# dnbaker/bonsai

Hardware: AMD Instinct MI355X
Metric: reads/s classified (150 bp) (higher is better)
Workload: dtype u64

## Files before the change

### bonsai_amd/csrc/bns_device.hpp

```cpp
#pragma once
#include <hip/hip_runtime.h>
#include <stdint.h>
#include <type_traits>

namespace bns {

using u8 = uint8_t;
using u16 = uint16_t;
using u32 = uint32_t;
using u64 = uint64_t;

constexpr u32 TAX_ABSENT = 0xFFFFFFFFu;

struct alignas(16) Slot {
    u64 key;
    u32 val;
    u32 occ;
};

struct alignas(16) TaxNode {
    u32 parent;
    u32 tin, tout;
    u32 flags;
};
constexpr u32 NODE_PRESENT = 1u, NODE_CHAIN_OK = 2u;

__device__ __forceinline__ int lane_id() { return (int)(threadIdx.x & 63u); }

__device__ __forceinline__ u64 wang64(u64 key)
{
    key = (~key) + (key << 21);
    key = key ^ (key >> 24);
    key = (key + (key << 3)) + (key << 8);
    key = key ^ (key >> 14);
    key = (key + (key << 2)) + (key << 4);
    key = key ^ (key >> 28);
    key = key + (key << 31);
    return key;
}

__device__ __forceinline__ u32 pairswap_not(u32 x)
{
    u32 r;
    const u32 c = 0x55555555u;
    asm("v_bitop3_b32 %0, %1, %2, %3 bitop3:0x1b" : "=v"(r) : "v"(x >> 1), "v"(x << 1), "s"(c));
    return r;
}
__device__ __forceinline__ u64 revcomp(u64 kmer, u32 k)
{
    const u32 a = __builtin_bitreverse32((u32)(kmer >> 32)), b = __builtin_bitreverse32((u32)kmer);
    const u32 lo = pairswap_not(a), hi = pairswap_not(b);
    return (((u64)hi << 32) | lo) >> (64u - (k << 1));
}

__device__ __forceinline__ u64 revcomp_top(u64 win, u32 k)
{
    const u32 a = __builtin_bitreverse32((u32)(win >> 32)), b = __builtin_bitreverse32((u32)win);
    const u32 lo = pairswap_not(a), hi = pairswap_not(b);
    return (((u64)hi << 32) | lo) & (~0ULL >> (64u - (k << 1)));
}

__device__ __forceinline__ u64 canonical(u64 kmer, u32 k)
{
    const u64 rc = revcomp(kmer, k);
    return kmer < rc ? kmer : rc;
}

template <int CTRL>
__device__ __forceinline__ u32 dpp(u32 v)
{
    return (u32)__builtin_amdgcn_update_dpp(0, (int)v, CTRL, 0xf, 0xf, true);
}
template <int CTRL>
__device__ __forceinline__ u64 dpp64(u64 v)
{
    const u32 lo = dpp<CTRL>((u32)v), hi = dpp<CTRL>((u32)(v >> 32));
    return ((u64)hi << 32) | lo;
}
constexpr int QP_XOR1 = 0xB1;
constexpr int QP_XOR2 = 0x4E;
template <int S> struct QBcast { static constexpr int ctrl = S * 0x55; };

__device__ __forceinline__ u64 ballot64(bool p) { return __builtin_amdgcn_ballot_w64(p); }
__device__ __forceinline__ u32 readlane(u32 v, int l) { return (u32)__builtin_amdgcn_readlane((int)v, l); }
__device__ __forceinline__ u64 readlane64(u64 v, int l)
{
    return ((u64)readlane((u32)(v >> 32), l) << 32) | readlane((u32)v, l);
}
__device__ __forceinline__ u64 lanemask_lt() { return (1ULL << lane_id()) - 1ULL; }

struct ProbeResult { u32 val; bool found; };
#ifdef BNS_COUNT_FETCHES
__device__ unsigned long long g_fetch_count[8];
#endif

__device__ __forceinline__ ProbeResult probe_khash(const u32 *__restrict__ flags, const u64 *__restrict__ keys,
                                                   const u32 *__restrict__ vals, u64 n_buckets, u64 key, bool active)
{
    ProbeResult r{0u, false};
    if (!active || n_buckets == 0) return r;
    const u64 mask = n_buckets - 1;
    u64 i = wang64(key) & mask, step = 0;
    const u64 last = i;
    for (;;) {
        const u32 f = (flags[i >> 4] >> ((i & 0xfu) << 1)) & 3u;
        if (f & 2u) return r;
        if (!(f & 1u) && keys[i] == key) { r.val = vals[i]; r.found = true; return r; }
        i = (i + (++step)) & mask;
        if (i == last) return r;
    }
}

// ... 293 lines not shown
    if (!PEEL || pass(std::true_type{}))
        while (more && pass(std::false_type{})) {}
#ifdef BNS_COUNT_FETCHES
    { const u64 g2 = ballot64(found == 2u); if (g2 && lane == 0) { atomicAdd(&g_fetch_count[2], (unsigned long long)__popcll(g2)); atomicAdd(&g_fetch_count[3], 1ULL); } }
#endif
    if (OVF_COOP) {
        bool go = found == 2u;
        u64 todo = ballot64(go);
        if (todo) {
            u32 *lb = aux, *lstep = aux + 16, *lres = aux + 32, *lflag = aux + 48;
            u64 *lkey = reinterpret_cast<u64 *>(aux + MINB_LIST_U32);
            const uint4 *ob = reinterpret_cast<const uint4 *>(ovf_slots);
            u32 l3 = (u32)lane;
            asm volatile("" : "+v"(l3));
            const u32 q = (l3 >> 2) & 15u, sub = l3 & 3u;
            do {
                const u32 rank = __builtin_amdgcn_mbcnt_hi((u32)(todo >> 32), __builtin_amdgcn_mbcnt_lo((u32)todo, 0u));
                const bool mine = go && rank < 16u;
                const u32 n = (u32)__popcll(todo);
                if (mine) { lkey[rank] = key; lb[rank] = (u32)ovf_bucket(key, ovf_mask); lstep[rank] = 0u; lflag[rank] = 0u; }
                __builtin_amdgcn_wave_barrier();
                bool walking = q < n;
                while (ballot64(walking)) {
                    u32 b = 0;
                    uint4 sl = make_uint4(0u, 0u, 0u, 0u);
                    if (walking) { b = lb[q]; sl = ob[(u64)b * 4u + sub]; }
                    const bool occ = sl.w != 0u;
                    const bool match = walking && occ && ((((u64)sl.y << 32) | sl.x) == lkey[q]);
                    u32 mv = match ? sl.z : 0u, fl = (match ? 1u : 0u) | (occ ? 2u : 0u);
                    mv |= dpp<QP_XOR1>(mv); mv |= dpp<QP_XOR2>(mv);
                    { const u32 o1 = dpp<QP_XOR1>(fl); fl = ((fl | o1) & 1u) | (fl & o1 & 2u); }
                    { const u32 o2 = dpp<QP_XOR2>(fl); fl = ((fl | o2) & 1u) | (fl & o2 & 2u); }
                    if (walking && sub == 0u) {
                        if (fl & 1u) { lres[q] = mv; lflag[q] = 1u; }
                        else if (fl & 2u) { const u32 st = lstep[q] + 1u; lstep[q] = st; lb[q] = (u32)(((u64)b + st) & ovf_mask); }
                    }
                    walking = walking && fl == 2u;
                    __builtin_amdgcn_wave_barrier();
                }
                if (mine && lflag[rank]) { found = 1u; val = lres[rank]; }
                go = go && !mine;
                todo = ballot64(go);
                __builtin_amdgcn_wave_barrier();
            } while (todo);
        }
        return ProbeResult{val, (found & 1u) != 0u};
    }
    minb_ovf_walk(key, found, val, ovf_slots, ovf_mask);
    ProbeResult r{val, (found & 1u) != 0u};
    return r;
}

constexpr int MINB_NB_WIDE = 24;
template <bool KEY_MAY_BE_ONES = true, int NB = 16>
__device__ __forceinline__ void probe_minbucket2(const MinBucket *__restrict__ buckets, u64 keyA, u32 bA, bool activeA, u64 keyB, u32 bB,
                                                 bool activeB, u32 *aux, const Slot *__restrict__ ovf_slots, u64 ovf_mask,
                                                 ProbeResult &ra, ProbeResult &rb, u32 nb = 16u)
{
    static_assert(NB == 16, "the two-key probe is built on a 16-bucket stage (two 1 KiB loads; nb = 24 adds a third)");
    const int lane = lane_id();
    u32 *list = aux;
    uint4 *stage = reinterpret_cast<uint4 *>(aux + MINB_LIST_U32);
    const uint4 *base = reinterpret_cast<const uint4 *>(buckets);
    u32 bktA = activeA ? bA : MINB_NONE, bktB = activeB ? bB : MINB_NONE;
    u32 foundA = 0u, valA = 0u, homeA = 0u, foundB = 0u, valB = 0u, homeB = 0u;
    const u32 xfA = mph_fold(keyA), xfB = mph_fold(keyB);
    constexpr u32 GO = 1u << MINB_HOME_SHIFT;
    auto look = [&](auto first_tag, u32 &bkt, u32 rank, u32 xf, u64 key, u32 &found, u32 &val, u32 home, u32 &hx) -> bool {
        constexpr bool FIRST = decltype(first_tag)::value;
        const bool mine = bkt != MINB_NONE && rank < nb;
        const char *B = reinterpret_cast<const char *>(stage) + (mine ? rank : 0u) * (16u * MINB_STRIDE);
        const uint2 hdr = *reinterpret_cast<const uint2 *>(B + 120);
        const u32 slot = mph_slot(xf, hdr.y);
        const bool eq = *reinterpret_cast<const u64 *>(B + 8u * slot) == key;
        const bool hit = mine & eq & (!KEY_MAY_BE_ONES || ((hdr.x >> (8u + slot)) & 1u));
        const u32 v = *reinterpret_cast<const u32 *>(B + 80 + 4u * slot);
        found = hit ? 1u : found;
        val = hit ? v : val;
        bool cont;
        if (FIRST) cont = mine & !hit & ((hdr.x & (GO | 0xFFu)) >= (GO | MINB_CAP));
        else       cont = mine & !hit & ((hdr.x & 0xFFu) >= MINB_CAP) & ((((home ? home : hdr.x) & GO)) != 0u);
        bkt = (mine && !cont) ? MINB_NONE : bkt;
        hx = hdr.x;
        return cont;
    };
    auto walk = [&](auto first_tag, bool cont, u32 hx, u32 &bkt, u32 &found, u32 &home) {
        constexpr bool FIRST = decltype(first_tag)::value;
        const u32 cur = (FIRST || home == 0u) ? ((hx & MINB_HOME_MASK) | (GO << 4)) : home;
        const bool exhausted = cont && (cur >> (MINB_HOME_SHIFT + 2u)) == 0u;
        found |= (exhausted || (cont && (hx & 0xFFu) == MINB_N_IN_OVF)) ? 2u : 0u;
        const u32 next = exhausted ? MINB_NONE : bkt + 1u;
        bkt = cont ? next : bkt;
        home = cont ? cur >> 1 : home;
    };
    bool more = true;
#ifdef BNS_COUNT_FETCHES
    u32 why_later = 4u;
#endif
    auto pass = [&](auto first_tag) -> bool {
        const u32 a63 = readlane(bktA, 63);
        const u32 prevA = (u32)__builtin_amdgcn_update_dpp((int)~bktA, (int)bktA, DPP_WAVE_SHR1, 0xf, 0xf, false);
        const u32 prevB = (u32)__builtin_amdgcn_update_dpp((int)a63, (int)bktB, DPP_WAVE_SHR1, 0xf, 0xf, false);
        const bool pendA = bktA != MINB_NONE, chgA = bktA != prevA, pendB = bktB != MINB_NONE, chgB = bktB != prevB;
        const u64 leadA = ballot64(pendA) & ballot64(chgA), leadB = ballot64(pendB) & ballot64(chgB);
        if (!(leadA | leadB)) return false;
        const u32 nA = (u32)__popcll(leadA);
        const int n_lead = (int)nA + __popcll(leadB);
#ifdef BNS_COUNT_FETCHES
        if (lane == 0) {
            atomicAdd(&g_fetch_count[0], (unsigned long long)((u32)n_lead < nb ? (u32)n_lead : nb)); atomicAdd(&g_fetch_count[1], 1ULL);
            if (!decltype(first_tag)::value) atomicAdd(&g_fetch_count[why_later], 1ULL);
        }
#endif
        const u32 rankA = __builtin_amdgcn_mbcnt_hi((u32)(leadA >> 33), __builtin_amdgcn_mbcnt_lo((u32)(leadA >> 1), (u32)(leadA & 1ULL) - 1u));
        const u32 rankB = __builtin_amdgcn_mbcnt_hi((u32)(leadB >> 33), __builtin_amdgcn_mbcnt_lo((u32)(leadB >> 1), nA + (u32)(leadB & 1ULL) - 1u));
        if (pendA & chgA) list[rankA] = bktA;
        if ((pendB & chgB) && rankB < nb) list[rankB] = bktB;
        __builtin_amdgcn_wave_barrier();
        {
            const u32 last = (u32)n_lead - 1u, slot = (u32)lane >> 3;
            typedef const void __attribute__((address_space(1))) *gptr_t;
            typedef void __attribute__((address_space(3))) *lptr_t;
            const u32 b0 = list[slot < last ? slot : last];
            __builtin_amdgcn_global_load_lds((gptr_t)(base + ((u64)b0 * 8 + (u64)(lane & 7))), (lptr_t)stage, 16, 0, 2);
            if (last >= 8u) {
                const u32 b1 = list[slot + 8u < last ? slot + 8u : last];
                __builtin_amdgcn_global_load_lds((gptr_t)(base + ((u64)b1 * 8 + (u64)(lane & 7))), (lptr_t)(stage + 64), 16, 0, 2);
                if (last >= 16u && nb > 16u) {
                    const u32 b2 = list[slot + 16u < last ? slot + 16u : last];
                    __builtin_amdgcn_global_load_lds((gptr_t)(base + ((u64)b2 * 8 + (u64)(lane & 7))), (lptr_t)(stage + 128), 16, 0, 2);
                }
            }
            asm volatile("s_waitcnt vmcnt(0)" ::: "memory");
        }
        __builtin_amdgcn_wave_barrier();
        u32 hxA, hxB;
        const bool contA = look(first_tag, bktA, rankA, xfA, keyA, foundA, valA, homeA, hxA);
        const bool contB = look(first_tag, bktB, rankB, xfB, keyB, foundB, valB, homeB, hxB);
        const u64 cA = ballot64(contA), cB = ballot64(contB);
        more = (u32)n_lead > nb || (cA | cB) != 0ULL;
#ifdef BNS_COUNT_FETCHES
        why_later = 4u + ((u32)n_lead > nb ? 1u : 0u) + ((cA | cB) != 0ULL ? 2u : 0u);
#endif
        if (cA) walk(first_tag, contA, hxA, bktA, foundA, homeA);
        if (cB) walk(first_tag, contB, hxB, bktB, foundB, homeB);
        __builtin_amdgcn_wave_barrier();
        return true;
    };
    if (pass(std::true_type{}))
        while (more && pass(std::false_type{})) {}
#ifdef BNS_COUNT_FETCHES
    { const u64 gA = ballot64(foundA == 2u), gB = ballot64(foundB == 2u);
      if ((gA | gB) && lane == 0) { atomicAdd(&g_fetch_count[2], (unsigned long long)(__popcll(gA) + __popcll(gB))); atomicAdd(&g_fetch_count[3], 1ULL); } }
#endif
    minb_ovf_walk(keyA, foundA, valA, ovf_slots, ovf_mask);
    minb_ovf_walk(keyB, foundB, valB, ovf_slots, ovf_mask);
    ra = ProbeResult{valA, (foundA & 1u) != 0u};
    rb = ProbeResult{valB, (foundB & 1u) != 0u};
}

__device__ __forceinline__ TaxNode load_node(const TaxNode *__restrict__ nodes, u32 n_nodes, u32 id)
{
    if (id < n_nodes) return nodes[id];
    return TaxNode{TAX_ABSENT, 0u, 0u, 0u};
}

__device__ __forceinline__ bool anc_or_self(u32 x, const TaxNode &nx, u32 a, const TaxNode &na)
{
    return x == a || (nx.tin < na.tin && na.tin < nx.tout);
// ... 20 lines not shown
```

### bonsai_amd/csrc/bns_kernels.hip

```cpp
#include "bns_device.hpp"
#include "bns_kernels.hpp"

namespace bns {

typedef const volatile __attribute__((address_space(4))) ClassifyParams ColdParams;
__device__ __forceinline__ ColdParams *cold_params() { return (ColdParams *)__builtin_amdgcn_kernarg_segment_ptr(); }

__device__ __forceinline__ u32 base_code(u32 b, u32 &bad)
{
    const u32 c = b & 0xDFu;
    const bool ok = (c == 0x41u) | (c == 0x43u) | (c == 0x47u) | (c == 0x54u);
    const u32 x = (c >> 1) & 3u;
    bad = ok ? 0u : 1u;
    return ok ? (x ^ (x >> 1)) : 0u;
}

__global__ __launch_bounds__(256) void pack_kernel(const u8 *__restrict__ bases, const u64 *__restrict__ offsets,
                                                   u64 n_reads, u64 *__restrict__ words, u32 *__restrict__ nmask)
{
    const int lane = lane_id();
    const u64 wave = (u64)blockIdx.x * (blockDim.x >> 6) + (u64)__builtin_amdgcn_readfirstlane((int)(threadIdx.x >> 6));
    const u64 n_waves = (u64)gridDim.x * (blockDim.x >> 6);
    for (u64 r = wave; r < n_reads; r += n_waves) {
        const u64 o = offsets[r];
// ... 111 lines not shown
    if (PACKED) asm volatile("" : "+v"(f.lo), "+v"(f.hi), "+v"(f.m));
    else        asm volatile("" : "+v"(f.lo), "+v"(f.hi));
}
template <bool PACKED>
__device__ __forceinline__ void prefetch_issue(const ClassifyParams &p, u64 r, u64 o, u32 L, Prefetch &f)
{
    if (!PACKED) { raw_load<true>(p.bases, o, L, 0u, f.lo, f.hi); return; }
    const u32 lane = (u32)lane_id();
    if (lane < ((L + 31u) >> 5)) {
        const u64 wi = (o >> 5) + r + lane;
        const u64 w = p.words[wi];
        f.lo = (u32)w; f.hi = (u32)(w >> 32);
        if (p.nmask) f.m = p.nmask[wi];
    }
}
__device__ __forceinline__ u64 mask1_to_mask2(u32 m)
{
    u64 x = m;
    x = (x | (x << 16)) & 0x0000FFFF0000FFFFULL;
    x = (x | (x << 8)) & 0x00FF00FF00FF00FFULL;
    x = (x | (x << 4)) & 0x0F0F0F0F0F0F0F0FULL;
    x = (x | (x << 2)) & 0x3333333333333333ULL;
    x = (x | (x << 1)) & 0x5555555555555555ULL;
    return x * 3ULL;
}
template <bool ORD32 = false>
__device__ __forceinline__ bool load_chunk_packed(const ClassifyParams &p, u64 r, u64 o, u32 L, u32 j0, bool have, const Prefetch &f, u64 *pk)
{
    const u32 lane = (u32)lane_id();
    u64 w = ((u64)f.hi << 32) | f.lo;
    u32 m = f.m;
    if (!have) {
        w = 0; m = 0;
        const u32 wl = (j0 >> 5) + lane;
        if (wl < ((L + 31u) >> 5)) {
            const u64 wi = (o >> 5) + r + wl;
            w = p.words[wi];
            if (p.nmask) m = p.nmask[wi];
        }
    }
    const bool dirty = ballot64(m != 0u) != 0ULL;
    if (ORD32) {
        u32 *img = reinterpret_cast<u32 *>(pk);
        img[1u + 2u * lane] = (u32)(w >> 32); img[2u + 2u * lane] = (u32)w;
        if (dirty) { const u64 m2 = mask1_to_mask2(m); img[IMG_N32 + 1u + 2u * lane] = (u32)(m2 >> 32); img[IMG_N32 + 2u + 2u * lane] = (u32)m2; }
    } else {
        pk[lane] = w;
        if (dirty) pk[64 + lane] = mask1_to_mask2(m);
    }
    __builtin_amdgcn_wave_barrier();
    return !dirty;
}

__device__ __forceinline__ void extract_lds32(const u64 *pk, u32 rd, u32 k, bool clean, u64 &win, bool &valid)
{
    const u32 lane = (u32)lane_id();
    const u32 *img = reinterpret_cast<const u32 *>(pk);
    const u32 g = 4u * rd + ((lane + 15u) >> 4), n = 30u - 2u * ((lane + 15u) & 15u);
    const u32 w0 = img[g], w1 = img[g + 1u], w2 = img[g + 2u];
    const u32 hi = __builtin_amdgcn_alignbit(w0, w1, n), lo = __builtin_amdgcn_alignbit(w1, w2, n);
    win = ((u64)hi << 32) | lo;
    valid = true;
    if (!clean) {
        const u32 m0 = img[IMG_N32 + g], m1 = img[IMG_N32 + g + 1u], m2 = img[IMG_N32 + g + 2u];
        const u64 mw = ((u64)__builtin_amdgcn_alignbit(m0, m1, n) << 32) | __builtin_amdgcn_alignbit(m1, m2, n);
        valid = (mw >> (64u - 2u * k)) == 0;
    }
}

__device__ __forceinline__ u32 mask2_to_mask1(u64 m2)
{
    u64 x = m2 & 0x5555555555555555ULL;
    x = (x | (x >> 1)) & 0x3333333333333333ULL;
    x = (x | (x >> 2)) & 0x0F0F0F0F0F0F0F0FULL;
    x = (x | (x >> 4)) & 0x00FF00FF00FF00FFULL;
    x = (x | (x >> 8)) & 0x0000FFFF0000FFFFULL;
    x = (x | (x >> 16)) & 0x00000000FFFFFFFFULL;
    return (u32)x;
}

__device__ __forceinline__ bool extract_unspaced(u64 W, u32 M, u32 rd, u32 k, u64 &kmer)
{
    const int lane = lane_id();
    const int w0 = (int)(2 * rd);
    const u64 wa = readlane64(W, w0), wb = readlane64(W, w0 + 1), wc = readlane64(W, w0 + 2);
    const u32 ma = readlane(M, w0), mb = readlane(M, w0 + 1), mc = readlane(M, w0 + 2);
    const bool up = lane >= 32;
    const u64 hi = up ? wb : wa, lo = up ? wc : wb;
    const u64 m64 = up ? (((u64)mb << 32) | mc) : (((u64)ma << 32) | mb);
    const u32 o = (u32)lane & 31u;
    const u64 win = o ? ((hi << (2 * o)) | (lo >> (64 - 2 * o))) : hi;
    kmer = win >> (64u - 2u * k);
    return ((m64 << o) >> (64u - k)) == 0;
}

template <int CTRL>
__device__ __forceinline__ u32 dpp_keep(u32 v)
{
    return (u32)__builtin_amdgcn_update_dpp(-1, (int)v, CTRL, 0xf, 0xf, false);
}
__device__ __forceinline__ u32 row_prefix_min(u32 x)
{
    x = min(x, dpp_keep<0x111>(x)); x = min(x, dpp_keep<0x112>(x)); x = min(x, dpp_keep<0x114>(x)); x = min(x, dpp_keep<0x118>(x));
    return x;
}
__device__ __forceinline__ u32 row_suffix_min(u32 x)
{
    x = min(x, dpp_keep<0x101>(x)); x = min(x, dpp_keep<0x102>(x)); x = min(x, dpp_keep<0x104>(x)); x = min(x, dpp_keep<0x108>(x));
    return x;
}
__device__ __forceinline__ u32 window16_min(u32 mine, u32 head, u32 rd, u32 *ring)
{
    const u32 lane = (u32)lane_id();
    if (rd == 0) {
        asm volatile("");
        const u32 sh = row_suffix_min(lane < 15u ? head : 0xFFFFFFFFu);
        if (lane < 15u) ring[lane] = sh;
    }
    const u32 P = row_prefix_min(mine), S = row_suffix_min(mine);
    ring[15u + lane] = S;
    __builtin_amdgcn_wave_barrier();
    const u32 sprev = ring[lane];
    __builtin_amdgcn_wave_barrier();
    if (lane >= 49u) ring[lane - 49u] = S;
    return min(P, sprev);
}

template <int W, bool VH = false>
__device__ __forceinline__ u32 round_minhash(u64 kf, u64 rc, u32 rd, u32 k, u32 m, u32 *ring)
{
    const int lane = lane_id();
    const u32 span = k - m;
    const u64 mmask = ~0ULL >> (64u - 2u * m);
    if (span == 0) { const u64 a = kf & mmask, b = rc & mmask; return mmer_hash(a < b ? a : b); }
    u32 mine;
    if (VH) {
        u32 head = 0;
        if (m <= 16u) {
            const u32 mm = 0xFFFFFFFFu >> (32u - 2u * m);
            if (rd == 0) head = mmer_mix(min((u32)(kf >> 30) & mm, (u32)rc & mm));
            mine = mmer_mix(min((u32)kf & mm, (u32)(rc >> 30)));
        } else {
            if (rd == 0) { const u64 a = kf >> 30, b = rc & mmask; head = mmer_hash(a < b ? a : b); }
            const u64 a = kf & mmask, b = rc >> 30;
            mine = mmer_hash(a < b ? a : b);
        }
        return window16_min(mine, head, rd, ring);
    }
    if (m <= 16u) {
        const u32 mm = 0xFFFFFFFFu >> (32u - 2u * m);
        if (rd == 0) { asm volatile(""); if ((u32)lane < span) ring[lane] = mmer_mix(min((u32)(kf >> (2u * span)) & mm, (u32)rc & mm)); }
        mine = mmer_mix(min((u32)kf & mm, (u32)(rc >> (2u * span))));
        ring[span + (u32)lane] = mine;
    } else {
        if (rd == 0) {
            if ((u32)lane < span) {
                const u64 a = kf >> (2u * span), b = rc & mmask;
                ring[lane] = mmer_hash(a < b ? a : b);
            }
        }
        const u64 a = kf & mmask, b = rc >> (2u * span);
        mine = mmer_hash(a < b ? a : b);
        ring[span + (u32)lane] = mine;
    }
    __builtin_amdgcn_wave_barrier();
    constexpr u32 G = W <= 9 ? (u32)W : ((u32)W + 1u) / 2u;
    u32 best = 0xFFFFFFFFu;
#pragma unroll
    for (u32 g = 0; g < (u32)W; g += G) {
        u32 h[G + 1];
#pragma unroll
        for (u32 i = 0; i <= G; ++i) h[i] = (i < G && g + i < (u32)W) ? ring[(u32)lane + g + i] : 0xFFFFFFFFu;
        if (span == (u32)W - 1u) {
#pragma unroll
            for (u32 i = 0; i < G; i += 2) if (g + i < (u32)W) best = min(min(best, h[i]), h[i + 1]);
        } else {
#pragma unroll
            for (u32 i = 0; i < G; ++i) { const u32 x = g + i <= span ? h[i] : 0xFFFFFFFFu; best = x < best ? x : best; }
        }
        if (g + G < (u32)W) { asm volatile("" : "+v"(best)); __builtin_amdgcn_sched_barrier(0); }
    }
    __builtin_amdgcn_wave_barrier();
    if ((u32)lane >= 64u - span) ring[(u32)lane + span - 64u] = mine;
    return best;
}

template <int W>
__device__ __forceinline__ u64 round_minhash_wide(u64 kf, u64 rc, u32 rd, u32 k, u32 m, u64 *ring)
{
    const int lane = lane_id();
    const u32 span = k - m;
    const u64 mmask = ~0ULL >> (64u - 2u * m);
    u64 mine;
    if (m <= 16u) {
        const u32 mm = 0xFFFFFFFFu >> (32u - 2u * m);
        if (span && rd == 0 && (u32)lane < span) ring[lane] = wide_ident32(min((u32)(kf >> (2u * span)) & mm, (u32)rc & mm));
        mine = wide_ident32(min((u32)kf & mm, (u32)(rc >> (2u * span)) & mm));
    } else {
        if (span && rd == 0 && (u32)lane < span) { const u64 a = kf >> (2u * span), b = rc & mmask; ring[lane] = wide_ident64(a < b ? a : b); }
        const u64 a = kf & mmask, b = rc >> (2u * span);
// ... 331 lines not shown
        best = s > best ? s : best;
    }
#pragma unroll
    for (int off = 32; off >= 1; off >>= 1) {
        const u32 o = (u32)__shfl_xor((int)best, off);
        best = o > best ? o : best;
    }
    u32 acc = 0;
    bool first = true;
    for (u32 base = 0; base < D; base += 64) {
        const u32 i = base + (u32)lane;
        const u32 s = i < D ? score_of(keys, cnt, tin, tout, D, i) : 0u;
        u64 tie = ballot64(i < D && s == best);
        while (tie) {
            const int l = __builtin_ctzll(tie);
            tie &= tie - 1;
            const u32 t = keys[base + (u32)l];
            if (first) { acc = t; first = false; }
            else acc = lca_dev(nodes, n_nodes, acc, t);
        }
    }
    return acc;
}

__device__ __forceinline__ u32 resolve_regs(u32 ckey, u32 ccnt, u32 D, const TaxNode *__restrict__ nodes, u32 n_nodes)
{
    const u32 lane = (u32)lane_id();
    const bool in = lane < D;
    u32 mytin = 0, mytout = 0;
    if (in) { const TaxNode nd = load_node(nodes, n_nodes, ckey); mytin = nd.tin; mytout = nd.tout; }
    u32 s = 0;
    for (u32 j = 0; j < D; ++j) {
        const u32 tj = readlane(ckey, (int)j), tinj = readlane(mytin, (int)j), toutj = readlane(mytout, (int)j);
        const u32 cj = readlane(ccnt, (int)j) & 0xFFFFu;
        const bool anc = (tj == ckey) ? (ckey != 0u) : (tinj < mytin && mytin < toutj);
        s += anc ? cj : 0u;
    }
    s = in ? s : 0u;
    u32 best = 0;
    for (u32 j = 0; j < D; ++j) { const u32 sj = readlane(s, (int)j); best = sj > best ? sj : best; }
    u64 tie = ballot64(in && s == best);
    u32 acc = 0;
    bool first = true;
    while (tie) {
        const int l = __builtin_ctzll(tie);
        tie &= tie - 1;
        const u32 t = readlane(ckey, l);
        if (first) { acc = t; first = false; }
        else acc = lca_dev(nodes, n_nodes, acc, t);
    }
    return acc;
}

template <bool SPACED, int LAYOUT, int KT, int NM, int NB = 16, int SPAN = 8, bool OVC = false, bool WIDE = false, bool PACKED = false, bool STAGE3 = false, class IssueNext>
__device__ __forceinline__ void classify_unit(const ClassifyParams &p, u64 u, u64 offv, u32 ob, bool have0, const Prefetch &pre0,
                                              u32 *keys, u32 *cnt, u32 *tin, u32 *tout, u32 cap, bool record_overflow, u32 *ring, u32 *aux, u64 *pk,
                                              uint4 &rec_out, bool &rec_valid, IssueNext &&issue_next)
{
    const int lane = lane_id();
    const u32 rdesc = SPACED ? run_desc(p) : 0u;
    const u32 k = KT ? (u32)KT : p.k, c = KT ? (u32)KT : p.c;
    const u32 mlen = KT ? (u32)(KT - SPAN) : p.m;
    constexpr int MW = KT ? SPAN + 1 : BNS_MAX_SPAN + 1;
    const int nm = NM ? NM : p.nmates;
    u32 D = 0, n_hits = 0, missing = 0, ambig = 0;
    u32 ckey = 0, ccnt = 0;
    u64 dmask = 0;
    bool overflow = false;
    const bool want_hits = p.want_hits != 0;
    const u32 rounds_per_chunk = (2048u - (c - 1u)) / 64u;
    u32 n_mb = p.n_mb;
    asm volatile("" : "+s"(n_mb));

    Prefetch pre1{0u, 0u, 0u};
    const bool have1 = !SPACED && NM == 2 && !OVC;
#ifdef BNS_PAD_UNIT
    { u32 pv = (u32)lane; for (int q = 0; q < BNS_PAD_UNIT; ++q) asm volatile("v_mul_lo_u32 %0, %0, %0" : "+v"(pv)); asm volatile("" :: "v"(pv)); }
#endif
    constexpr bool PAIRS = !SPACED && LAYOUT == 2 && KT != 0 && !OVC && !WIDE;
    auto tally = [&](const ProbeResult &pr, bool valid) -> u64 {
        const u64 fm = ballot64(pr.found), vm = ballot64(valid);
        missing += (u32)__popcll(vm & ~fm);
        if (want_hits && pr.found) { u32 *hp = cold_params()->hits; hp[readlane64(offv, (int)ob) + n_hits + (u32)__popcll(fm & lanemask_lt())] = pr.val; }
        n_hits += (u32)__popcll(fm);
        return fm;
    };
    auto vote2 = [&](u64 fa, u32 va, u64 fb, u32 vb) {
        u64 ra = fa, rb = fb;
        while (ra | rb) {
            const bool inA = ra != 0ULL;
            const int l = __builtin_ctzll(inA ? ra : rb);
            const u32 t = readlane(inA ? va : vb, l);
            const u64 ma = ballot64(va == t) & ra, mb = ballot64(vb == t) & rb;
            ra &= ~ma; rb &= ~mb;
            const u32 c = (u32)(__popcll(ma) + __popcll(mb));
            const bool eq = ckey == t;
            if (ballot64(eq) & dmask) { ccnt = eq ? ccnt + c : ccnt; continue; }
            if (!counter_insert(ckey, ccnt, dmask, keys, cnt, cap, D, t, c)) { overflow = true; break; }
        }
    };
    auto pack = [&](int m, u32 L, u32 j0, bool have, const Prefetch &pre) __attribute__((always_inline)) -> bool {
        return PACKED ? load_chunk_packed<!SPACED>(p, u * (u64)nm + (u64)m, readlane64(offv, (int)ob + m), L, j0, have, pre, pk)
                      : pack_chunk_lds<!SPACED>(p.bases, offv, (int)ob + m, L, j0, have, pre.lo, pre.hi, pk);
    };
    auto n_kmers = [&](u32 L) -> u32 { return (L >= c && !(SPACED && p.emit_none)) ? L - c + 1u : 0u; };
    bool clean0 = true;
    {
        const u32 L = readlane((u32)offv, (int)ob + 1) - readlane((u32)offv, (int)ob);
        if (n_kmers(L)) clean0 = pack(0, L, 0u, have0, pre0);
        if (have1) prefetch_clear<PACKED>(pre1);
        issue_next();
        if (have1) prefetch_issue<PACKED>(p, u * (u64)nm + 1u, readlane64(offv, (int)ob + 1), readlane((u32)offv, (int)ob + 2) - readlane((u32)offv, (int)ob + 1), pre1);
    }
    for (int m = 0; m < nm; ++m) {
        const u32 L = readlane((u32)offv, (int)ob + m + 1) - readlane((u32)offv, (int)ob + m);
        const u32 nk = n_kmers(L);
        for (u32 j0 = 0; j0 < nk; j0 += rounds_per_chunk * 64u) {
            const bool clean = (m == 0 && j0 == 0u) ? clean0 : pack(m, L, j0, have1 && m != 0 && j0 == 0u, pre1);
            u64 W = 0; u32 M = 0xFFFFFFFFu;
            if (SPACED) {
                const u32 n_written = PACKED ? 64u : ((L - j0 >= 2048u ? 2048u : L - j0) + 255u) / 256u * 8u;
                W = (u32)lane < n_written ? pk[lane] : 0ULL;
                if (!p.n_runs) M = (PACKED && clean) ? 0u : mask2_to_mask1((u32)lane < n_written ? pk[64 + lane] : ~0ULL);
            }
            const u32 chunk_nk = (nk - j0) < rounds_per_chunk * 64u ? (nk - j0) : rounds_per_chunk * 64u;
            if constexpr (PAIRS) {
                auto key_round = [&](u32 rd, u64 &key, u32 &bkt) -> bool {
                    u64 win = 0;
                    bool valid;
                    extract_lds32(pk, rd, k, clean, win, valid);
                    const u64 kf = win >> (64u - 2u * k), krc = revcomp_top(win, k);
                    key = kf < krc ? kf : krc;
                    bkt = bucket_of(round_minhash<MW, SPAN == 15>(kf, krc, rd, k, mlen, ring), n_mb);
                    return valid && rd * 64u + (u32)lane < chunk_nk;
                };
                for (u32 rd = 0; rd * 64u < chunk_nk; rd += 2u) {
                    u64 keyA;
                    u32 bA;
                    const bool vA = key_round(rd, keyA, bA);
                    if ((rd + 1u) * 64u < chunk_nk) {
                        u64 keyB;
                        u32 bB;
                        const bool vB = key_round(rd + 1u, keyB, bB);
                        ProbeResult pa, pb;
                        probe_minbucket2<(KT == 32), NB>(p.minb, keyA, bA, vA, keyB, bB, vB, aux, p.slots, p.ovf_mask, pa, pb,
                                                         (STAGE3 && D <= 64u) ? (u32)MINB_NB_WIDE : 16u);
                        const u64 fa = tally(pa, vA), fb = tally(pb, vB);
                        vote2(fa, pa.val, fb, pb.val);
                    } else {
                        const ProbeResult pa = probe_minbucket<(KT == 32), NB>(p.minb, keyA, bA, vA, aux, p.slots, p.ovf_mask);
                        vote2(tally(pa, vA), pa.val, 0ULL, 0u);
                    }
                }
                continue;
            }
            for (u32 rd = 0; rd * 64u < chunk_nk; ++rd) {
                const u32 jl = rd * 64u + (u32)lane;
                u64 kmer, win = 0;
                bool valid;
                if (SPACED) valid = p.n_runs ? extract_spaced_lds(pk, rd, p, rdesc, kmer, clean) : extract_spaced(W, M, rd, k, rdesc, kmer);
                else        { extract_lds32(pk, rd, k, clean, win, valid); kmer = win >> (64u - 2u * k); }
                valid = valid && jl < chunk_nk;
#ifdef BNS_PAD_VALU
                { u32 pv = (u32)lane; for (int q = 0; q < BNS_PAD_VALU; ++q) asm volatile("v_mul_lo_u32 %0, %0, %0" : "+v"(pv)); asm volatile("" :: "v"(pv)); }
#endif
#ifdef BNS_PAD_VFAST
                { u32 pv = (u32)lane; for (int q = 0; q < BNS_PAD_VFAST; ++q) asm volatile("v_add_u32 %0, %0, %0" : "+v"(pv)); asm volatile("" :: "v"(pv)); }
#endif
#ifdef BNS_PAD_SALU
                { for (int q = 0; q < BNS_PAD_SALU; ++q) asm volatile("s_add_u32 s20, s20, 3" ::: "s20", "scc"); }
#endif
#ifdef BNS_PAD_LDS
                { u32 pv; for (int q = 0; q < BNS_PAD_LDS; ++q) asm volatile("ds_read_b32 %0, %1" : "=v"(pv) : "v"((u32)lane * 4u)); asm volatile("s_waitcnt lgkmcnt(0)" ::: "memory"); }
#endif
                const u64 kf = kmer;
                const u64 krc = SPACED ? 0ULL : revcomp_top(win, k);
                if (!SPACED && (KT != 0 || p.canon)) kmer = kf < krc ? kf : krc;
                ProbeResult pr;
#ifdef BNS_ABLATION
                if (p.dbg & 1) { pr.found = valid && (kmer & 1); pr.val = 1000u + (u32)(kmer & 3); }
                else
#endif
                if (LAYOUT == 2) {
                    u32 minh;
                    if (SPACED) minh = key_minhash(kmer, k, MinSpec{p.m, p.min_len, p.min_shift, p.min_canon, 0u});
                    else if (WIDE) minh = wide_bucket_in(round_minhash_wide<MW>(kf, krc, rd, k, mlen, reinterpret_cast<u64 *>(ring)), mlen);
                    else minh = round_minhash<MW, (KT != 0 && SPAN == 15)>(kf, krc, rd, k, mlen, ring);
#ifdef BNS_ABLATION
// ... 21 lines not shown
                }
            }
        }
        if (m == 0) ambig = L - c + 1u - n_hits - missing;
        else        ambig += L - (c - 1u) - n_hits - missing;
    }

    ColdParams *kp = cold_params();
    if (overflow && record_overflow) {
        if (lane == 0) {
            u32 *oc = kp->ovf_count;
            u64 *ol = kp->ovf_list;
            if (ol) { const u32 slot = atomicAdd(oc, 1u); ol[slot] = u; }
        }
        rec_valid = false;
        return;
    }
    u32 taxon;
    if (D <= 1u) taxon = D ? readlane(ckey, 0) : 0u;
    else if (D <= 64u) taxon = resolve_regs(ckey, ccnt, D, kp->nodes, kp->n_nodes);
    else {
        u32 l2 = (u32)lane;
        asm volatile("" : "+v"(l2));
        keys[l2] = ckey; cnt[l2] = ccnt;
        __builtin_amdgcn_wave_barrier();
        taxon = resolve_wave(keys, cnt, tin, tout, D, kp->nodes, kp->n_nodes, (int)(l2 & 63u));
    }
    rec_out = make_uint4(taxon, missing, ambig, n_hits);
    rec_valid = true;
}

#ifndef BNS_WAVES_PER_SIMD
#define BNS_WAVES_PER_SIMD 8
#endif
#ifdef BNS_WAVE_TIMES
__device__ unsigned long long g_wave_times[2 * 8192];
#endif
#ifndef BNS_SPACED_NB
#define BNS_SPACED_NB 32
#endif
#ifndef BNS_SPACED_WAVES
#define BNS_SPACED_WAVES 6
#endif
template <bool SPACED> struct ClassifyCfg { static constexpr int NB = 16, WAVES = BNS_WAVES_PER_SIMD; };
template <> struct ClassifyCfg<true> { static constexpr int NB = BNS_SPACED_NB, WAVES = BNS_SPACED_WAVES; };
template <bool SPACED, int LAYOUT, int KT, int NM, int SPAN = 8, bool OVC = false, bool WIDE = false, bool PACKED = false>
__global__ __launch_bounds__(256, (LAYOUT == 1 && !SPACED) ? 7 : ClassifyCfg<SPACED>::WAVES) void classify_kernel(ClassifyParams p)
{
    constexpr int NB = LAYOUT == 2 ? ClassifyCfg<SPACED>::NB : 16;
    constexpr bool PAIRS = !SPACED && LAYOUT == 2 && KT != 0 && !OVC && !WIDE;
    constexpr int AUX_U32 = PAIRS ? minb_aux_u32(MINB_NB_WIDE) : minb_aux_u32(NB);
    constexpr bool STAGE3 = PAIRS && !(NM == 2 && !PACKED);
    static_assert(!PAIRS || (NB == 16 && minb_aux_u32(MINB_NB_WIDE) == minb_aux_u32(16) + 2 * (int)LDS_CAP), "the counter is the stage's third KiB");
    __shared__ __attribute__((aligned(8))) u32 s_ring[4][WIDE ? 160 : 96];
    __shared__ __attribute__((aligned(16))) u32 s_mh[4][AUX_U32];
    __shared__ u64 s_pk[4][IMG_U64];
    static_assert(AUX_U32 - MINB_LIST_U32 >= 2 * (int)LDS_CAP, "stage must hold tin/tout");
    const int wv = __builtin_amdgcn_readfirstlane((int)(threadIdx.x >> 6));
    u32 *ctr_keys, *ctr_cnt;
    if constexpr (PAIRS) {
        ctr_keys = s_mh[wv] + minb_aux_u32(16); ctr_cnt = ctr_keys + LDS_CAP;
    } else {
        __shared__ u32 s_keys[4][LDS_CAP], s_cnt[4][LDS_CAP];
        ctr_keys = s_keys[wv]; ctr_cnt = s_cnt[wv];
    }
    const int lane = lane_id();
#ifdef BNS_WAVE_TIMES
    const unsigned long long t_start = wall_clock64();
    struct TimeStamp { unsigned long long t0; u32 slot; __device__ ~TimeStamp() { if ((threadIdx.x & 63u) == 0) { g_wave_times[2 * slot] = t0; g_wave_times[2 * slot + 1] = wall_clock64(); } } } stamp{t_start, blockIdx.x * 4u + (u32)wv};
#endif
    const u32 n_units = (u32)p.n_units;
    const u32 nm = NM ? (u32)NM : (u32)p.nmates;
    u32 *const ctr = p.work_counter;
    const u32 CH = p.chunk;
    auto claim = [&]() -> u32 { return lane == 0 ? atomicAdd(ctr, CH) : 0u; };
    auto load_offs = [&](u32 base) -> u64 {
        const u32 left = n_units - base, cnt = left < CH ? left : CH;
        const u64 *op = const_cast<const u64 *>(cold_params()->offsets) + (u64)base * nm;
        return (u32)lane <= cnt * nm ? op[lane] : 0ULL;
    };
    u32 base = (u32)__builtin_amdgcn_readfirstlane((int)claim());
    if (base >= n_units) return;
    u64 offs = load_offs(base);
    Prefetch pre;
    {
        const u64 o0 = readlane64(offs, 0);
        prefetch_clear<PACKED>(pre);
        prefetch_issue<PACKED>(p, (u64)base * nm, o0, readlane((u32)offs, 1) - (u32)o0, pre);
    }
    uint4 pend = make_uint4(0, 0, 0, 0);
    u32 pend_u = 0;
    bool pend_valid = false;
    for (;;) {
        const u32 left = n_units - base, cnt = left < CH ? left : CH;
        u32 next_v = claim();
        u32 nbase = 0xFFFFFFFFu;
        u64 noffs = 0;
        const u32 jload = cnt > 2u ? 2u : cnt - 1u;
        for (u32 j = 0; j < cnt; ++j) {
            if (j == jload) {
                nbase = (u32)__builtin_amdgcn_readfirstlane((int)next_v);
                if (nbase < n_units) noffs = load_offs(nbase);
            }
            Prefetch npre;
            auto issue_next = [&]() __attribute__((always_inline)) {
                prefetch_clear<PACKED>(npre);
                u64 n0 = 0, nr = 0;
// ... 936 lines not shown
```

Baseline: 1.984 billion.

## Assign adjacent k-mer pairs per lane for paired minimizer bucket probing

For contiguous k-mers with k<=31, each lane now takes two adjacent k-mers (2*lane, 2*lane+1) instead of one from each of two 64-wide rounds. Both k-mers come from one shared window extraction and one reverse complement, and a paired minimizer computes both hashes with new DPP block-of-8 prefix/suffix scans. The probe's leader detection compares B against A in the same lane, which makes duplicate buckets between neighbouring k-mers cheaper to find. This aims to cut extraction, revcomp and minimizer work and improve bucket dedup, at the cost of a larger LDS ring and new tally and vote paths.

```diff
diff --git a/bonsai_amd/csrc/bns_device.hpp b/bonsai_amd/csrc/bns_device.hpp
--- a/bonsai_amd/csrc/bns_device.hpp
+++ b/bonsai_amd/csrc/bns_device.hpp
@@ -58,6 +58,13 @@
     const u32 a = __builtin_bitreverse32((u32)(win >> 32)), b = __builtin_bitreverse32((u32)win);
     const u32 lo = pairswap_not(a), hi = pairswap_not(b);
     return (((u64)hi << 32) | lo) & (~0ULL >> (64u - (k << 1)));
+}
+
+__device__ __forceinline__ u64 revcomp64(u64 win)
+{
+    const u32 a = __builtin_bitreverse32((u32)(win >> 32)), b = __builtin_bitreverse32((u32)win);
+    const u32 lo = pairswap_not(a), hi = pairswap_not(b);
+    return ((u64)hi << 32) | lo;
 }
 
 __device__ __forceinline__ u64 canonical(u64 kmer, u32 k)
@@ -457,7 +464,7 @@
 }
 
 constexpr int MINB_NB_WIDE = 24;
-template <bool KEY_MAY_BE_ONES = true, int NB = 16>
+template <bool KEY_MAY_BE_ONES = true, int NB = 16, bool ADJ = false>
 __device__ __forceinline__ void probe_minbucket2(const MinBucket *__restrict__ buckets, u64 keyA, u32 bA, bool activeA, u64 keyB, u32 bB,
                                                  bool activeB, u32 *aux, const Slot *__restrict__ ovf_slots, u64 ovf_mask,
                                                  ProbeResult &ra, ProbeResult &rb, u32 nb = 16u)
@@ -503,13 +510,21 @@
     u32 why_later = 4u;
 #endif
     auto pass = [&](auto first_tag) -> bool {
-        const u32 a63 = readlane(bktA, 63);
-        const u32 prevA = (u32)__builtin_amdgcn_update_dpp((int)~bktA, (int)bktA, DPP_WAVE_SHR1, 0xf, 0xf, false);
-        const u32 prevB = (u32)__builtin_amdgcn_update_dpp((int)a63, (int)bktB, DPP_WAVE_SHR1, 0xf, 0xf, false);
-        const bool pendA = bktA != MINB_NONE, chgA = bktA != prevA, pendB = bktB != MINB_NONE, chgB = bktB != prevB;
-        const u64 leadA = ballot64(pendA) & ballot64(chgA), leadB = ballot64(pendB) & ballot64(chgB);
+        bool pendA, chgA, pendB, chgB;
+        u64 leadA, leadB;
+        u32 nA;
+        if constexpr (ADJ) {
+            const u32 prevA = (u32)__builtin_amdgcn_update_dpp((int)~bktA, (int)bktB, DPP_WAVE_SHR1, 0xf, 0xf, false);
+            pendA = bktA != MINB_NONE; chgA = bktA != prevA; pendB = bktB != MINB_NONE; chgB = bktB != bktA;
+        } else {
+            const u32 a63 = readlane(bktA, 63);
+            const u32 prevA = (u32)__builtin_amdgcn_update_dpp((int)~bktA, (int)bktA, DPP_WAVE_SHR1, 0xf, 0xf, false);
+            const u32 prevB = (u32)__builtin_amdgcn_update_dpp((int)a63, (int)bktB, DPP_WAVE_SHR1, 0xf, 0xf, false);
+            pendA = bktA != MINB_NONE; chgA = bktA != prevA; pendB = bktB != MINB_NONE; chgB = bktB != prevB;
+        }
+        leadA = ballot64(pendA) & ballot64(chgA); leadB = ballot64(pendB) & ballot64(chgB);
         if (!(leadA | leadB)) return false;
-        const u32 nA = (u32)__popcll(leadA);
+        nA = (u32)__popcll(leadA);
         const int n_lead = (int)nA + __popcll(leadB);
 #ifdef BNS_COUNT_FETCHES
         if (lane == 0) {
@@ -517,9 +532,16 @@
             if (!decltype(first_tag)::value) atomicAdd(&g_fetch_count[why_later], 1ULL);
         }
 #endif
-        const u32 rankA = __builtin_amdgcn_mbcnt_hi((u32)(leadA >> 33), __builtin_amdgcn_mbcnt_lo((u32)(leadA >> 1), (u32)(leadA & 1ULL) - 1u));
-        const u32 rankB = __builtin_amdgcn_mbcnt_hi((u32)(leadB >> 33), __builtin_amdgcn_mbcnt_lo((u32)(leadB >> 1), nA + (u32)(leadB & 1ULL) - 1u));
-        if (pendA & chgA) list[rankA] = bktA;
+        u32 rankA, rankB;
+        if constexpr (ADJ) {
+            const u32 upA = __builtin_amdgcn_mbcnt_hi((u32)(leadA >> 33), __builtin_amdgcn_mbcnt_lo((u32)(leadA >> 1), (u32)(leadA & 1ULL) - 1u));
+            rankA = __builtin_amdgcn_mbcnt_hi((u32)(leadB >> 32), __builtin_amdgcn_mbcnt_lo((u32)leadB, upA));
+            rankB = rankA + ((pendB & chgB) ? 1u : 0u);
+        } else {
+            rankA = __builtin_amdgcn_mbcnt_hi((u32)(leadA >> 33), __builtin_amdgcn_mbcnt_lo((u32)(leadA >> 1), (u32)(leadA & 1ULL) - 1u));
+            rankB = __builtin_amdgcn_mbcnt_hi((u32)(leadB >> 33), __builtin_amdgcn_mbcnt_lo((u32)(leadB >> 1), nA + (u32)(leadB & 1ULL) - 1u));
+        }
+        if ((pendA & chgA) && (!ADJ || rankA < nb)) list[rankA] = bktA;
         if ((pendB & chgB) && rankB < nb) list[rankB] = bktB;
         __builtin_amdgcn_wave_barrier();
         {
diff --git a/bonsai_amd/csrc/bns_kernels.hip b/bonsai_amd/csrc/bns_kernels.hip
--- a/bonsai_amd/csrc/bns_kernels.hip
+++ b/bonsai_amd/csrc/bns_kernels.hip
@@ -187,9 +187,8 @@
     return !dirty;
 }
 
-__device__ __forceinline__ void extract_lds32(const u64 *pk, u32 rd, u32 k, bool clean, u64 &win, bool &valid)
-{
-    const u32 lane = (u32)lane_id();
+__device__ __forceinline__ void extract_lds32(const u64 *pk, u32 rd, u32 k, bool clean, u64 &win, bool &valid, u32 lane = (u32)lane_id())
+{
     const u32 *img = reinterpret_cast<const u32 *>(pk);
     const u32 g = 4u * rd + ((lane + 15u) >> 4), n = 30u - 2u * ((lane + 15u) & 15u);
     const u32 w0 = img[g], w1 = img[g + 1u], w2 = img[g + 2u];
@@ -244,9 +243,8 @@
     x = min(x, dpp_keep<0x101>(x)); x = min(x, dpp_keep<0x102>(x)); x = min(x, dpp_keep<0x104>(x)); x = min(x, dpp_keep<0x108>(x));
     return x;
 }
-__device__ __forceinline__ u32 window16_min(u32 mine, u32 head, u32 rd, u32 *ring)
-{
-    const u32 lane = (u32)lane_id();
+__device__ __forceinline__ u32 window16_min(u32 mine, u32 head, u32 rd, u32 *ring, u32 lane = (u32)lane_id())
+{
     if (rd == 0) {
         asm volatile("");
         const u32 sh = row_suffix_min(lane < 15u ? head : 0xFFFFFFFFu);
@@ -261,10 +259,101 @@
     return min(P, sprev);
 }
 
+__device__ __forceinline__ void extract_lds32_adj(const u64 *pk, u32 q, u32 k, bool clean, u64 &win, bool &okA, bool &okB)
+{
+    const u32 lane = (u32)lane_id();
+    const u32 *img = reinterpret_cast<const u32 *>(pk);
+    const u32 g = 8u * q + ((2u * lane + 15u) >> 4), n = 30u - 2u * ((2u * lane + 15u) & 15u);
+    const u32 w0 = img[g], w1 = img[g + 1u], w2 = img[g + 2u];
+    win = ((u64)__builtin_amdgcn_alignbit(w0, w1, n) << 32) | __builtin_amdgcn_alignbit(w1, w2, n);
+    okA = true; okB = true;
+    if (!clean) {
+        const u32 m0 = img[IMG_N32 + g], m1 = img[IMG_N32 + g + 1u], m2 = img[IMG_N32 + g + 2u];
+        const u64 mw = ((u64)__builtin_amdgcn_alignbit(m0, m1, n) << 32) | __builtin_amdgcn_alignbit(m1, m2, n);
+        okA = (mw >> (64u - 2u * k)) == 0;
+        okB = ((mw << 2) >> (64u - 2u * k)) == 0;
+    }
+}
+
+__device__ __forceinline__ u32 blk8_prefix_min(u32 x)
+{
+    x = min(x, dpp<0x90>(x));
+    x = min(x, dpp<0x44>(x));
+    const u32 t = dpp<0xFF>(x);
+    return min(x, (u32)__builtin_amdgcn_update_dpp(-1, (int)t, 0x114, 0xf, 0xa, false));
+}
+__device__ __forceinline__ u32 blk8_suffix_min(u32 x)
+{
+    x = min(x, dpp<0xF9>(x));
+    x = min(x, dpp<0xEE>(x));
+    const u32 t = dpp<0x00>(x);
+    return min(x, (u32)__builtin_amdgcn_update_dpp(-1, (int)t, 0x104, 0xf, 0x5, false));
+}
+__device__ __forceinline__ u32 blk8_exclusive(u32 inc, bool prefix)
+{
+    u32 r;
+    if (prefix) {
+        const u32 t = dpp<0x111>(inc);
+        asm("s_mov_b32 vcc_lo, 0x01010101\n\ts_mov_b32 vcc_hi, 0x01010101\n\tv_cndmask_b32_e64 %0, %1, -1, vcc" : "=v"(r) : "v"(t) : "vcc");
+    } else {
+        const u32 t = dpp<0x101>(inc);
+        asm("s_mov_b32 vcc_lo, 0x80808080\n\ts_mov_b32 vcc_hi, 0x80808080\n\tv_cndmask_b32_e64 %0, %1, -1, vcc" : "=v"(r) : "v"(t) : "vcc");
+    }
+    return r;
+}
+
+__device__ __forceinline__ void window16_min2(u32 h0, u32 h1, u32 g0, u32 g1, u32 *ring, u32 &wA, u32 &wB)
+{
+    const u32 lane = (u32)lane_id();
+    uint2 *ring2 = reinterpret_cast<uint2 *>(ring);
+    const u32 Xv = blk8_suffix_min(min(g0, g1));
+    ring2[lane] = make_uint2(Xv, min(Xv, dpp<0x111>(g1)));
+    __builtin_amdgcn_wave_barrier();
+    const u32 pm = min(h0, h1);
+    const u32 P = blk8_prefix_min(pm), S = blk8_suffix_min(pm);
+    ring2[8u + lane] = make_uint2(min(h1, blk8_exclusive(S, false)), S);
+    __builtin_amdgcn_wave_barrier();
+    const u32 xin = ring[2u * lane], sin = ring[2u * lane + 3u];
+    __builtin_amdgcn_wave_barrier();
+    wA = min(min(xin, blk8_exclusive(P, true)), h0);
+    wB = min(sin, P);
+}
+
+template <int SPAN>
+__device__ __forceinline__ void round2_minhash(u64 kfA, u64 rcA, u64 kfB, u64 rcB, u32 m, u32 *ring, u32 &hA, u32 &hB)
+{
+    static_assert(SPAN >= 2, "a window of at least three m-mers");
+    const u32 lane = (u32)lane_id();
+    const u64 mmask = ~0ULL >> (64u - 2u * m);
+    auto canon_hash = [&](u64 a, u64 b) -> u32 {
+        if (m <= 16u) return mmer_mix(min((u32)a, (u32)b));
+        return mmer_hash(a < b ? a : b);
+    };
+    const u32 g0 = canon_hash(kfA >> (2u * SPAN), rcA & mmask), g1 = canon_hash(kfB >> (2u * SPAN), rcB & mmask);
+    const u32 h0 = canon_hash(kfA & mmask, rcA >> (2u * SPAN)), h1 = canon_hash(kfB & mmask, rcB >> (2u * SPAN));
+    if (SPAN == 15) { window16_min2(h0, h1, g0, g1, ring, hA, hB); return; }
+    u32 c = min(g1, h0);
+    constexpr u32 NP = ((u32)SPAN - 1u) / 2u;
+    if (NP) {
+        uint2 *ring2 = reinterpret_cast<uint2 *>(ring);
+        ring2[lane] = make_uint2(g0, g1);
+        ring[2u * lane + (u32)SPAN] = h0; ring[2u * lane + (u32)SPAN + 1u] = h1;
+        __builtin_amdgcn_wave_barrier();
+        uint2 h[NP ? NP : 1u];
+#pragma unroll
+        for (u32 i = 0; i < NP; ++i) h[i] = ring2[lane + 1u + i];
+#pragma unroll
+        for (u32 i = 0; i < NP; ++i) c = min(min(c, h[i].x), h[i].y);
+        __builtin_amdgcn_wave_barrier();
+    }
+    hA = min(c, g0);
+    hB = min(c, h1);
+}
+
 template <int W, bool VH = false>
-__device__ __forceinline__ u32 round_minhash(u64 kf, u64 rc, u32 rd, u32 k, u32 m, u32 *ring)
-{
-    const int lane = lane_id();
+__device__ __forceinline__ u32 round_minhash(u64 kf, u64 rc, u32 rd, u32 k, u32 m, u32 *ring, u32 lane_ = (u32)lane_id())
+{
+    const int lane = (int)lane_;
     const u32 span = k - m;
     const u64 mmask = ~0ULL >> (64u - 2u * m);
     if (span == 0) { const u64 a = kf & mmask, b = rc & mmask; return mmer_hash(a < b ? a : b); }
@@ -280,7 +369,7 @@
             const u64 a = kf & mmask, b = rc >> 30;
             mine = mmer_hash(a < b ? a : b);
         }
-        return window16_min(mine, head, rd, ring);
+        return window16_min(mine, head, rd, ring, lane_);
     }
     if (m <= 16u) {
         const u32 mm = 0xFFFFFFFFu >> (32u - 2u * m);
@@ -718,6 +807,8 @@
     return acc;
 }
 
+constexpr bool adjacent_kmers(int kt, int span) { return kt != 0 && kt <= 31 && span >= 2; }
+constexpr int ring_u32(bool wide, bool adj) { return wide ? 160 : (adj ? 144 : 96); }
 template <bool SPACED, int LAYOUT, int KT, int NM, int NB = 16, int SPAN = 8, bool OVC = false, bool WIDE = false, bool PACKED = false, bool STAGE3 = false, class IssueNext>
 __device__ __forceinline__ void classify_unit(const ClassifyParams &p, u64 u, u64 offv, u32 ob, bool have0, const Prefetch &pre0,
                                               u32 *keys, u32 *cnt, u32 *tin, u32 *tout, u32 cap, bool record_overflow, u32 *ring, u32 *aux, u64 *pk,
@@ -744,6 +835,7 @@
     { u32 pv = (u32)lane; for (int q = 0; q < BNS_PAD_UNIT; ++q) asm volatile("v_mul_lo_u32 %0, %0, %0" : "+v"(pv)); asm volatile("" :: "v"(pv)); }
 #endif
     constexpr bool PAIRS = !SPACED && LAYOUT == 2 && KT != 0 && !OVC && !WIDE;
+    constexpr bool ADJ = PAIRS && adjacent_kmers(KT, SPAN);
     auto tally = [&](const ProbeResult &pr, bool valid) -> u64 {
         const u64 fm = ballot64(pr.found), vm = ballot64(valid);
         missing += (u32)__popcll(vm & ~fm);
@@ -765,6 +857,30 @@
             if (!counter_insert(ckey, ccnt, dmask, keys, cnt, cap, D, t, c)) { overflow = true; break; }
         }
     };
+    auto tally_adj = [&](const ProbeResult &pa, bool vA, const ProbeResult &pb, bool vB, u64 &fa, u64 &fb) {
+        fa = ballot64(pa.found); fb = ballot64(pb.found);
+        missing += (u32)(__popcll(ballot64(vA) & ~fa) + __popcll(ballot64(vB) & ~fb));
+        if (want_hits && (pa.found || pb.found)) {
+            u32 *hp = cold_params()->hits + (readlane64(offv, (int)ob) + n_hits + (u32)(__popcll(fa & lanemask_lt()) + __popcll(fb & lanemask_lt())));
+            if (pa.found) hp[0] = pa.val;
+            if (pb.found) hp[pa.found ? 1 : 0] = pb.val;
+        }
+        n_hits += (u32)(__popcll(fa) + __popcll(fb));
+    };
+    auto vote_adj = [&](u64 fa, u32 va, u64 fb, u32 vb) {
+        u64 ra = fa, rb = fb;
+        while (ra | rb) {
+            const int l = __builtin_ctzll(ra | rb);
+            const bool inA = ((ra >> l) & 1ULL) != 0ULL;
+            const u32 t = readlane(inA ? va : vb, l);
+            const u64 ma = ballot64(va == t) & ra, mb = ballot64(vb == t) & rb;
+            ra &= ~ma; rb &= ~mb;
+            const u32 c = (u32)(__popcll(ma) + __popcll(mb));
+            const bool eq = ckey == t;
+            if (ballot64(eq) & dmask) { ccnt = eq ? ccnt + c : ccnt; continue; }
+            if (!counter_insert(ckey, ccnt, dmask, keys, cnt, cap, D, t, c)) { overflow = true; break; }
+        }
+    };
     auto pack = [&](int m, u32 L, u32 j0, bool have, const Prefetch &pre) __attribute__((always_inline)) -> bool {
         return PACKED ? load_chunk_packed<!SPACED>(p, u * (u64)nm + (u64)m, readlane64(offv, (int)ob + m), L, j0, have, pre, pk)
                       : pack_chunk_lds<!SPACED>(p.bases, offv, (int)ob + m, L, j0, have, pre.lo, pre.hi, pk);
@@ -794,12 +910,45 @@
                 auto key_round = [&](u32 rd, u64 &key, u32 &bkt) -> bool {
                     u64 win = 0;
                     bool valid;
-                    extract_lds32(pk, rd, k, clean, win, valid);
+                    u32 lq = (u32)lane;
+                    if (ADJ) asm volatile("" : "+v"(lq));
+                    extract_lds32(pk, rd, k, clean, win, valid, lq);
                     const u64 kf = win >> (64u - 2u * k), krc = revcomp_top(win, k);
                     key = kf < krc ? kf : krc;
-                    bkt = bucket_of(round_minhash<MW, SPAN == 15>(kf, krc, rd, k, mlen, ring), n_mb);
-                    return valid && rd * 64u + (u32)lane < chunk_nk;
+                    bkt = bucket_of(round_minhash<MW, SPAN == 15>(kf, krc, ADJ ? 0u : rd, k, mlen, ring, lq), n_mb);
+                    return valid && rd * 64u + lq < chunk_nk;
                 };
+                if constexpr (ADJ) {
+                    for (u32 rd = 0; rd * 64u < chunk_nk; rd += 2u) {
+                        if ((rd + 1u) * 64u < chunk_nk) {
+                            u64 win;
+                            bool okA, okB;
+                            extract_lds32_adj(pk, rd >> 1, k, clean, win, okA, okB);
+                            const u64 kmask = ~0ULL >> (64u - 2u * k);
+                            const u64 rcw = revcomp64(win);
+                            const u64 kfA = win >> (64u - 2u * k), kfB = (win << 2) >> (64u - 2u * k);
+                            const u64 rcA = rcw & kmask, rcB = (rcw >> 2) & kmask;
+                            const u64 keyA = kfA < rcA ? kfA : rcA, keyB = kfB < rcB ? kfB : rcB;
+                            u32 hA, hB;
+                            round2_minhash<SPAN>(kfA, rcA, kfB, rcB, mlen, ring, hA, hB);
+                            const u32 left = chunk_nk - rd * 64u;
+                            const bool vA = okA && 2u * (u32)lane < left, vB = okB && 2u * (u32)lane < left - 1u;
+                            ProbeResult pa, pb;
+                            probe_minbucket2<false, NB, true>(p.minb, keyA, bucket_of(hA, n_mb), vA, keyB, bucket_of(hB, n_mb), vB, aux, p.slots, p.ovf_mask,
+                                                              pa, pb, (STAGE3 && D <= 64u) ? (u32)MINB_NB_WIDE : 16u);
+                            u64 fa, fb;
+                            tally_adj(pa, vA, pb, vB, fa, fb);
+                            vote_adj(fa, pa.val, fb, pb.val);
+                        } else {
+                            u64 keyA;
+                            u32 bA;
+                            const bool vA = key_round(rd, keyA, bA);
+                            const ProbeResult pa = probe_minbucket<false, NB>(p.minb, keyA, bA, vA, aux, p.slots, p.ovf_mask);
+                            vote2(tally(pa, vA), pa.val, 0ULL, 0u);
+                        }
+                    }
+                    continue;
+                }
                 for (u32 rd = 0; rd * 64u < chunk_nk; rd += 2u) {
                     u64 keyA;
                     u32 bA;
@@ -927,7 +1076,7 @@
     constexpr int AUX_U32 = PAIRS ? minb_aux_u32(MINB_NB_WIDE) : minb_aux_u32(NB);
     constexpr bool STAGE3 = PAIRS && !(NM == 2 && !PACKED);
     static_assert(!PAIRS || (NB == 16 && minb_aux_u32(MINB_NB_WIDE) == minb_aux_u32(16) + 2 * (int)LDS_CAP), "the counter is the stage's third KiB");
-    __shared__ __attribute__((aligned(8))) u32 s_ring[4][WIDE ? 160 : 96];
+    __shared__ __attribute__((aligned(8))) u32 s_ring[4][ring_u32(WIDE, PAIRS && adjacent_kmers(KT, SPAN))];
     __shared__ __attribute__((aligned(16))) u32 s_mh[4][AUX_U32];
     __shared__ u64 s_pk[4][IMG_U64];
     static_assert(AUX_U32 - MINB_LIST_U32 >= 2 * (int)LDS_CAP, "stage must hold tin/tout");
```

Result: faster. 2.049 billion, median of 6 (+3.3%).
